# mic-rud/Learned-Compression-of-Point-Cloud-Geometry-and-Attributes

Measured on AMD Instinct MI355X. Metric: encode+decode Mpoints/sec, higher is better.
Workload: dtype f32

## Files before the change

include/pcc_hip.h:

```cpp
#ifndef PCC_HIP_H
#define PCC_HIP_H

#include <stdint.h>

#ifdef __cplusplus
extern "C" {
#endif

#define PCC_OK 0
#define PCC_ERR_ARG (-1)
#define PCC_ERR_HIP (-2)
#define PCC_ERR_UNSUPPORTED (-3)
#define PCC_ERR_DATA (-4)

#define PCC_ACT_NONE 0
#define PCC_ACT_RELU 1
#define PCC_ACT_LEAKY_RELU 2

int pcc_version(void);
const char* pcc_last_error(void);
int pcc_device_count(void);
int pcc_device_name(int dev, char* out, int out_len);

int64_t pcc_hash_capacity(int64_t n);
// ... 34 lines not shown
int64_t pcc_small_map_max(void);
int32_t pcc_small_paths(int32_t mask);
int pcc_small_kernel_map(const int32_t* out_coords, int64_t n_out, const uint64_t* in_keys, const int32_t* in_vals, int64_t in_cap,
                         int32_t ksize, int32_t step, int32_t sign, int32_t* nbr, uint32_t* row_mask, int32_t* order,
                         uint32_t* group_mask32, void* scratch, int64_t scratch_bytes, void* stream);

int64_t pcc_conv_packed_elems(int32_t K, int32_t cin, int32_t cout);
int pcc_conv_pack_weights(const float* w, int32_t K, int32_t cin, int32_t cout, float* w_packed,
                          void* stream);
int pcc_conv_fwd(const float* fin, int64_t n_in, int32_t cin, const float* w, const float* w_packed,
                 const float* bias, const int32_t* nbr, const int32_t* order,
                 const uint32_t* group_mask32, int32_t K, float* fout, int64_t n_out, int32_t cout,
                 int32_t act, const float* film, const float* residual, void* stream);

int64_t pcc_conv_small_max(int64_t workgroups);

int pcc_conv_kernel_name(int32_t mode, int64_t n_in, int32_t cin, int32_t cout, int64_t n_out, int32_t K, int32_t has_nbr,
                         char* buf, int32_t len);

int64_t pcc_conv_packed_elems_bf16(int32_t K, int32_t cin, int32_t cout);
int pcc_conv_pack_weights_bf16(const float* w, int32_t K, int32_t cin, int32_t cout, uint16_t* w_packed, void* stream);
int pcc_conv_fwd_bf16(const uint16_t* fin, int64_t n_in, int32_t cin, const uint16_t* w_packed, const float* bias,
                      const int32_t* nbr, const int32_t* order, const uint32_t* group_mask32, int32_t K, float* fout,
                      int64_t n_out, int32_t cout, int32_t act, const float* film, const float* residual, void* stream);

int pcc_epilogue_fwd(const float* c, const float* film, const float* residual, int64_t n, int32_t channels, int32_t act,
                     float* out, void* stream);
int pcc_epilogue_bwd(const float* dout, const float* c, const float* film, int64_t n, int32_t channels, int32_t act,
                     float* dc, float* dfilm, void* stream);

// ... 118 lines not shown
```

learned-compression-of-point-cloud-geometry-and-attributes_amd/_lib.py:

```python
import ctypes
import os
import subprocess

_HERE = os.path.dirname(os.path.abspath(__file__))
SO_PATH = os.path.join(_HERE, "libpcc_hip.so")
_lib = None

c_void_p, c_int, c_i32, c_i64 = ctypes.c_void_p, ctypes.c_int, ctypes.c_int32, ctypes.c_int64

SIGNATURES = {
    "pcc_version": (c_int, []),
    "pcc_last_error": (ctypes.c_char_p, []),
    "pcc_device_count": (c_int, []),
    "pcc_device_name": (c_int, [c_int, ctypes.c_char_p, c_int]),
    "pcc_hash_capacity": (c_i64, [c_i64]),
    "pcc_hash_build": (c_int, [c_void_p, c_i64, c_void_p, c_void_p, c_i64, c_i32, c_void_p, c_void_p]),
    "pcc_hash_lookup": (c_int, [c_void_p, c_void_p, c_i64, c_i32, c_void_p, c_i64, c_void_p, c_void_p]),
    "pcc_scan_scratch_elems": (c_i64, [c_i64]),
    "pcc_stride_map": (c_int, [c_void_p, c_i64, c_i32, c_void_p, c_void_p, c_i64, c_void_p, c_void_p, c_void_p, c_void_p]),
    "pcc_children": (c_int, [c_void_p, c_i64, c_i32, c_i32, c_void_p, c_void_p, c_i64, c_void_p, c_void_p, c_void_p, c_void_p]),
    "pcc_kernel_map": (c_int, [c_void_p, c_i64, c_void_p, c_void_p, c_i64, c_i32, c_i32, c_i32, c_void_p, c_void_p, c_void_p, c_void_p]),
    "pcc_pair_count": (c_int, [c_void_p, c_i64, c_void_p, c_void_p]),
    "pcc_conv_packed_elems": (c_i64, [c_i32, c_i32, c_i32]),
    "pcc_conv_pack_weights": (c_int, [c_void_p, c_i32, c_i32, c_i32, c_void_p, c_void_p]),
    "pcc_order_scratch_bytes": (c_i64, [c_i64]),
    "pcc_order_rows_by_mask": (c_int, [c_void_p, c_void_p, c_i64, c_i32, c_i32, c_void_p, c_void_p, c_void_p, c_i64, c_void_p]),
    "pcc_permute_map_rows": (c_int, [c_void_p, c_void_p, c_i64, c_i32, c_void_p, c_void_p]),
    "pcc_conv_fwd": (c_int, [c_void_p, c_i64, c_i32, c_void_p, c_void_p, c_void_p, c_void_p, c_void_p, c_void_p, c_i32,
                             c_void_p, c_i64, c_i32, c_i32, c_void_p, c_void_p, c_void_p]),
    "pcc_conv_small_max": (c_i64, [c_i64]),
    "pcc_conv_kernel_name": (c_int, [c_i32, c_i64, c_i32, c_i32, c_i64, c_i32, c_i32, ctypes.c_char_p, c_i32]),
    "pcc_small_map_max": (c_i64, []),
    "pcc_small_paths": (c_i32, [c_i32]),
    "pcc_small_kernel_map": (c_int, [c_void_p, c_i64, c_void_p, c_void_p, c_i64, c_i32, c_i32, c_i32, c_void_p, c_void_p, c_void_p,
                                     c_void_p, c_void_p, c_i64, c_void_p]),
    "pcc_conv_packed_elems_bf16": (c_i64, [c_i32, c_i32, c_i32]),
    "pcc_conv_pack_weights_bf16": (c_int, [c_void_p, c_i32, c_i32, c_i32, c_void_p, c_void_p]),
    "pcc_conv_fwd_bf16": (c_int, [c_void_p, c_i64, c_i32, c_void_p, c_void_p, c_void_p, c_void_p, c_void_p, c_i32, c_void_p, c_i64,
                                  c_i32, c_i32, c_void_p, c_void_p, c_void_p]),
    "pcc_conv_packed_elems_x3": (c_i64, [c_i32, c_i32, c_i32]),
    "pcc_conv_pack_weights_x3": (c_int, [c_void_p, c_i32, c_i32, c_i32, c_void_p, c_void_p]),
    "pcc_conv_fwd_x3": (c_int, [c_void_p, c_i64, c_i32, c_void_p, c_void_p, c_void_p, c_void_p, c_void_p, c_i32, c_void_p, c_i64,
                                c_i32, c_i32, c_void_p, c_void_p, c_void_p]),
    "pcc_epilogue_fwd": (c_int, [c_void_p, c_void_p, c_void_p, c_i64, c_i32, c_i32, c_void_p, c_void_p]),
    "pcc_cast_colsum_scratch_elems": (c_i64, [c_i32]),
# ... 211 lines not shown
```

learned-compression-of-point-cloud-geometry-and-attributes_amd/csrc/conv.hip:

```cpp
#include <stdlib.h>

#include <type_traits>

#include "common.h"

namespace pcc {

typedef float f32x2 __attribute__((ext_vector_type(2)));
typedef float f32x4 __attribute__((ext_vector_type(4)));
typedef float f32x16 __attribute__((ext_vector_type(16)));
typedef __bf16 bf16x8 __attribute__((ext_vector_type(8)));

struct ConvArgs {
    const float* fin;
    const float* w;
    const float* wp;
    const float* bias;
    const int32_t* nbr;
    const int32_t* order;
    const uint32_t* gmask;
    float* fout;
    const float* film;
    const float* residual;
    int64_t n_in, n_out;
// ... 68 lines not shown
        wp[((base + 0 * 4 + g) * coutp + col) * 8 + j] = hi;
        wp[((base + 1 * 4 + g) * coutp + col) * 8 + j] = mid;
        wp[((base + 2 * 4 + g) * coutp + col) * 8 + j] = lo;
    }
}

constexpr int A_LD_DMA = 32;

template <int BM, int BN, bool X3 = false>
constexpr int conv_lds_bytes() { return 2 * (BM * A_LD_DMA + (X3 ? 12 : 8) * BN * 4) * (int)sizeof(float); }

__device__ float g_zero_line[256] = {0.0f};

typedef __attribute__((address_space(3))) void* lds_ptr_t;
typedef const __attribute__((address_space(1))) void* gbl_ptr_t;

template <int BM, int BN, int WAVES_M, int WAVES_N, bool HAS_NBR>
__global__ __launch_bounds__(256) void conv_mfma_kernel(const ConvArgs a) {
    constexpr int RPT = BM / 32;
    constexpr int WM = BM / WAVES_M, WN = BN / WAVES_N;
    constexpr int MT = WM / 32, NT = WN / 32;
    constexpr int A_LD = A_LD_DMA;
    constexpr int A_ELEMS = BM * A_LD;
    constexpr int W_ELEMS = 8 * BN * 4;
    constexpr int W_LOADS = (8 * BN) / 256;
    static_assert(WAVES_M * WAVES_N == 4 && MT >= 1 && NT >= 1 && W_LOADS >= 1, "bad tiling");

    extern __shared__ __attribute__((aligned(16))) float smem[];
    float* As = smem;
    float* Ws = smem + 2 * A_ELEMS;
// ... 232 lines not shown
    constexpr int W_ELEMS = (X3 ? 12 : 8) * BN * 4;
    constexpr int W_LOADS = ((X3 ? 12 : 8) * BN) / 256;
    static_assert(WAVES_M * WAVES_N == 4 && MT >= 1 && MT <= 2 && NT >= 1 && W_LOADS >= 1, "bad tiling");
    static_assert(!(BF16 && X3), "one operand mode at a time");
    constexpr int ESZ = BF16 ? 2 : 4;

    extern __shared__ __attribute__((aligned(16))) float smem[];
    float* As = smem;
    float* Ws = smem + 2 * A_ELEMS;

    const int t = threadIdx.x;
    const int lane = t & 63, wid = t >> 6;
    const int r = lane & 31, h = lane >> 5;
    const int wrow = (wid / WAVES_N) * WM, wcol = (wid % WAVES_N) * WN;

    const int ntiles_n = a.coutp / BN;
    const int64_t tile = blockIdx.x / ntiles_n;
    const int nt = blockIdx.x - (int)(tile * ntiles_n);
    const int64_t row0 = tile * BM;
    const int K = a.K;

    uint32_t tmask, mmask[MT];
    {
        const uint32_t all = (K >= 32) ? 0xffffffffu : ((1u << K) - 1u);
        if (a.gmask) {
            const int64_t g0 = row0 >> 5;
            const int64_t ng = (a.n_out + 31) >> 5;
            tmask = 0u;
#pragma unroll
            for (int g = 0; g < BM / 32; ++g) tmask |= (g0 + g < ng) ? (a.gmask[g0 + g] & all) : 0u;
#pragma unroll
            for (int m = 0; m < MT; ++m) {
                const int64_t g = g0 + (wrow >> 5) + m;
                const uint32_t v = (g < ng) ? (a.gmask[g] & all) : 0u;
                mmask[m] = __builtin_amdgcn_readfirstlane(v);
            }
        } else {
            tmask = all;
#pragma unroll
            for (int m = 0; m < MT; ++m) mmask[m] = all;
        }
        tmask = __builtin_amdgcn_readfirstlane(tmask);
    }

    f32x16 acc[MT][NT];
#pragma unroll
    for (int m = 0; m < MT; ++m)
#pragma unroll
        for (int n = 0; n < NT; ++n) {
#pragma unroll
            for (int i = 0; i < 16; ++i) acc[m][n][i] = 0.0f;
        }

    if (tmask != 0u) {
        __amdgpu_buffer_rsrc_t rsrc_a = __builtin_amdgcn_make_buffer_rsrc(
            const_cast<float*>(a.fin), 0, (int)(uint32_t)(a.n_in * a.cin * ESZ), BUF_FLAGS);
        __amdgpu_buffer_rsrc_t rsrc_w = __builtin_amdgcn_make_buffer_rsrc(
            const_cast<float*>(a.wp), 0, (int)((uint32_t)K * a.cin * a.coutp * (X3 ? 6 : ESZ)), BUF_FLAGS);
        __amdgpu_buffer_rsrc_t rsrc_n = __builtin_amdgcn_make_buffer_rsrc(
            const_cast<int32_t*>(a.nbr), 0, HAS_NBR ? (int)(uint32_t)(a.n_out * K * 4) : 0, BUF_FLAGS);

        const int gchunk = t & 7;
        uint32_t q16[RPT], n_voff[RPT], a_voff[RPT];
        int idx_nxt[RPT];
        bool rvalid[RPT];
#pragma unroll
        for (int i = 0; i < RPT; ++i) {
            const int grow = wid * (BM / 4) + 8 * i + (lane >> 3);
            const int64_t pos = row0 + grow;
            rvalid[i] = pos < a.n_out;
            const int64_t ps = rvalid[i] ? pos : a.n_out - 1;
            q16[i] = (uint32_t)((gchunk ^ ((grow >> 1) & 7)) * 16);
            n_voff[i] = (uint32_t)(((HAS_NBR && a.order) ? (int64_t)a.order[ps] : ps) * K * 4);
            idx_nxt[i] = (int)ps;
        }
        uint32_t w_voff[W_LOADS];
#pragma unroll
        for (int j = 0; j < W_LOADS; ++j) {
            const int f = t + 256 * j;
            const int g = f / BN, col = f - g * BN;
            w_voff[j] = (uint32_t)((g * a.coutp + nt * BN + col) * 16);
        }
        const int wave_u = __builtin_amdgcn_readfirstlane(wid);
        const uint32_t w_kstride = X3 ? (uint32_t)(a.cin / 32) * 12u * a.coutp * 16u
                                      : (uint32_t)(a.cin * ESZ / 16) * a.coutp * 16;
        const uint32_t w_cstride = (uint32_t)(X3 ? 12 : 8) * a.coutp * 16;
        const uint32_t a_row_bytes = (uint32_t)a.cin * ESZ;

        auto load_idx = [&](int k) {
            if constexpr (HAS_NBR) {
#pragma unroll
                for (int i = 0; i < RPT; ++i)
                    idx_nxt[i] = (int)__builtin_amdgcn_raw_buffer_load_b32(rsrc_n, n_voff[i], k * 4, 0);
            }
        };
        auto set_src = [&](bool real) {
#pragma unroll
            for (int i = 0; i < RPT; ++i) {
                const bool ok = real && rvalid[i] && idx_nxt[i] >= 0;
                a_voff[i] = ok ? (uint32_t)idx_nxt[i] * a_row_bytes + q16[i] : BUF_OOB;
            }
        };
        auto dma = [&](int k, auto cc, auto bufc) {
            constexpr int c = decltype(cc)::value;
            constexpr int buf = decltype(bufc)::value;
#pragma unroll
            for (int i = 0; i < RPT; ++i)
                __builtin_amdgcn_raw_ptr_buffer_load_lds(rsrc_a, (lds_ptr_t)(As + buf * A_ELEMS + (wave_u * RPT + i) * 256), 16,
                                                         a_voff[i], c * 128, 0, 0);
            const uint32_t wso = (uint32_t)k * w_kstride + (uint32_t)c * w_cstride;
#pragma unroll
            for (int j = 0; j < W_LOADS; ++j)
                __builtin_amdgcn_raw_ptr_buffer_load_lds(rsrc_w, (lds_ptr_t)(Ws + buf * W_ELEMS + (wave_u * 64 + 256 * j) * 4), 16,
                                                         w_voff[j], wso, 0, 0);
        };

        const int sw = (r >> 1) & 7;
        uint32_t a_addr[2][4], w_addr[2];
#pragma unroll
        for (int b = 0; b < 2; ++b) {
#pragma unroll
            for (int kk = 0; kk < 4; ++kk)
                a_addr[b][kk] = (uint32_t)((b * A_ELEMS + (wrow + r) * 32 + (((kk ^ (sw >> 1)) << 1) | (h ^ (sw & 1))) * 4) * 4);
            w_addr[b] = (uint32_t)((2 * A_ELEMS + b * W_ELEMS + (h * BN + wcol + r) * 4) * 4);
        }
        auto lds4 = [&](uint32_t addr) { return *reinterpret_cast<const f32x4*>(reinterpret_cast<const char*>(smem) + addr); };

        uint32_t a3_addr[2][2][2];
#pragma unroll
        for (int b = 0; b < 2; ++b)
#pragma unroll
            for (int q = 0; q < 2; ++q)
#pragma unroll
                for (int e = 0; e < 2; ++e)
                    a3_addr[b][q][e] = (uint32_t)((b * A_ELEMS + (wrow + r) * 32 + ((4 * q + 2 * h + e) ^ sw) * 4) * 4);
        auto split8 = [&](const f32x4& lo4, const f32x4& hi4, bf16x8& ph, bf16x8& pm, bf16x8& pl) {
            uint32_t hb[8], mb[8], lb[8];
#pragma unroll
            for (int j = 0; j < 8; ++j) {
                const float x = j < 4 ? lo4[j] : hi4[j - 4];
                hb[j] = __float_as_uint(x) & 0xFFFF0000u;
                const float r1 = x - __uint_as_float(hb[j]);
                mb[j] = __float_as_uint(r1) & 0xFFFF0000u;
                lb[j] = __float_as_uint(r1 - __uint_as_float(mb[j]));
            }
            typedef uint32_t u32x4 __attribute__((ext_vector_type(4)));
            u32x4 vh, vm, vl;
#pragma unroll
            for (int d = 0; d < 4; ++d) {
                vh[d] = __builtin_amdgcn_perm(hb[2 * d + 1], hb[2 * d], 0x07060302u);
                vm[d] = __builtin_amdgcn_perm(mb[2 * d + 1], mb[2 * d], 0x07060302u);
                vl[d] = __builtin_amdgcn_perm(lb[2 * d + 1], lb[2 * d], 0x07060302u);
            }
            ph = __builtin_bit_cast(bf16x8, vh);
            pm = __builtin_bit_cast(bf16x8, vm);
            pl = __builtin_bit_cast(bf16x8, vl);
        };
        auto compute_live_x3 = [&](auto bufc, auto live_tag) {
            constexpr int buf = decltype(bufc)::value;
            constexpr unsigned LIVE = decltype(live_tag)::value;
            __builtin_amdgcn_s_setprio(1);
#pragma unroll
            for (int q = 0; q < 2; ++q) {
                bf16x8 ah[MT], am[MT], al[MT];
#pragma unroll
                for (int m = 0; m < MT; ++m)
                    if ((LIVE >> m) & 1u)
                        split8(lds4(a3_addr[buf][q][0] + 32 * m * 32 * 4), lds4(a3_addr[buf][q][1] + 32 * m * 32 * 4), ah[m], am[m], al[m]);
                bf16x8 bh[NT], bm[NT], bl[NT];
#pragma unroll
                for (int n = 0; n < NT; ++n) {
                    const uint32_t wb = w_addr[buf] + (uint32_t)((2 * q * BN + 32 * n) * 16);
                    bh[n] = __builtin_bit_cast(bf16x8, lds4(wb));
                    bm[n] = __builtin_bit_cast(bf16x8, lds4(wb + 4 * BN * 16));
                    bl[n] = __builtin_bit_cast(bf16x8, lds4(wb + 8 * BN * 16));
                }
#define PCC_X3_TERM(A, B)                                                                                                   \
    _Pragma("unroll") for (int m = 0; m < MT; ++m) _Pragma("unroll") for (int n = 0; n < NT; ++n) if ((LIVE >> m) & 1u)     \
        acc[m][n] = __builtin_amdgcn_mfma_f32_32x32x16_bf16(A[m], B[n], acc[m][n], 0, 0, 0)
                PCC_X3_TERM(al, bh);
                PCC_X3_TERM(ah, bl);
                PCC_X3_TERM(am, bm);
                PCC_X3_TERM(am, bh);
                PCC_X3_TERM(ah, bm);
                PCC_X3_TERM(ah, bh);
#undef PCC_X3_TERM
            }
            __builtin_amdgcn_s_setprio(0);
        };
        auto compute_live = [&](auto bufc, auto live_tag) {
            if constexpr (X3) {
                compute_live_x3(bufc, live_tag);
                return;
            }
            constexpr int buf = decltype(bufc)::value;
            constexpr unsigned LIVE = decltype(live_tag)::value;
            f32x4 av[2][MT], bv[2][NT];
            __builtin_amdgcn_s_setprio(1);
#pragma unroll
            for (int m = 0; m < MT; ++m)
                if ((LIVE >> m) & 1u) av[0][m] = lds4(a_addr[buf][0] + 32 * m * 32 * 4);
#pragma unroll
            for (int n = 0; n < NT; ++n) bv[0][n] = lds4(w_addr[buf] + 32 * n * 16);
#pragma unroll
            for (int kk = 0; kk < 4; ++kk) {
                const int cb = kk & 1, nb = cb ^ 1;
                if (kk + 1 < 4) {
#pragma unroll
                    for (int m = 0; m < MT; ++m)
                        if ((LIVE >> m) & 1u) av[nb][m] = lds4(a_addr[buf][kk + 1] + 32 * m * 32 * 4);
#pragma unroll
                    for (int n = 0; n < NT; ++n) bv[nb][n] = lds4(w_addr[buf] + (2 * (kk + 1) * BN + 32 * n) * 16);
                }
                if constexpr (BF16) {
#pragma unroll
                    for (int m = 0; m < MT; ++m)
#pragma unroll
                        for (int n = 0; n < NT; ++n)
                            if ((LIVE >> m) & 1u)
                                acc[m][n] = __builtin_amdgcn_mfma_f32_32x32x16_bf16(__builtin_bit_cast(bf16x8, av[cb][m]),
                                                                                    __builtin_bit_cast(bf16x8, bv[cb][n]), acc[m][n], 0, 0, 0);
                } else {
#pragma unroll
                    for (int s = 0; s < 4; ++s)
#pragma unroll
                        for (int m = 0; m < MT; ++m)
#pragma unroll
                            for (int n = 0; n < NT; ++n)
                                if ((LIVE >> m) & 1u)
                                    acc[m][n] = __builtin_amdgcn_mfma_f32_32x32x2f32(av[cb][m][s], bv[cb][n][s], acc[m][n], 0, 0, 0);
                }
            }
            __builtin_amdgcn_s_setprio(0);
        };
        auto compute = [&](auto bufc, unsigned live) {
            if constexpr (MT == 1) {
                if (live) compute_live(bufc, std::integral_constant<unsigned, 1u>{});
            } else {
                if (live == 3u) compute_live(bufc, std::integral_constant<unsigned, 3u>{});
                else if (live == 1u) compute_live(bufc, std::integral_constant<unsigned, 1u>{});
                else if (live == 2u) compute_live(bufc, std::integral_constant<unsigned, 2u>{});
            }
        };

        uint32_t rem = tmask;
        int k = __builtin_ctz(rem);
        rem &= rem - 1u;
        auto offset_body = [&](auto pc) {
            constexpr int P = decltype(pc)::value;
            const int knext = rem ? __builtin_ctz(rem) : -1;
            const uint32_t rem2 = rem & (rem - 1u);
            const int kn2 = rem2 ? __builtin_ctz(rem2) : (knext >= 0 ? knext : k);
            unsigned live = 0;
#pragma unroll
            for (int m = 0; m < MT; ++m) live |= ((mmask[m] >> k) & 1u) << m;
            static_for<0, CCH>([&](auto cc) {
                constexpr int c = decltype(cc)::value;
                constexpr int buf = (P + c) & 1;
                if constexpr (c + 1 < CCH) {
                    dma(k, std::integral_constant<int, c + 1>{}, std::integral_constant<int, buf ^ 1>{});
                } else {
                    set_src(knext >= 0);
                    dma(knext >= 0 ? knext : k, std::integral_constant<int, 0>{}, std::integral_constant<int, buf ^ 1>{});
                    load_idx(kn2);
                }
                compute(std::integral_constant<int, buf>{}, live);
                __syncthreads();
            });
            const bool more = knext >= 0;
            k = more ? knext : k;
            rem = rem2;
            return more;
        };

        load_idx(k);
        set_src(true);
        dma(k, std::integral_constant<int, 0>{}, std::integral_constant<int, 0>{});
        load_idx(rem ? __builtin_ctz(rem) : k);
        __syncthreads();
        while (true) {
            if (!offset_body(std::integral_constant<int, 0>{})) break;
            if constexpr (CCH & 1) {
                if (!offset_body(std::integral_constant<int, 1>{})) break;
            }
        }
    }

#pragma unroll
    for (int m = 0; m < MT; ++m) {
#pragma unroll
        for (int n = 0; n < NT; ++n) {
#pragma unroll
            for (int reg = 0; reg < 16; ++reg) {
                const int col = nt * BN + wcol + 32 * n + r;
                if (col >= a.cout) continue;
                const float bcol = a.bias ? a.bias[col] : 0.0f;
                const int64_t pos = row0 + wrow + 32 * m + (reg & 3) + 8 * (reg >> 2) + 4 * h;
                if (pos >= a.n_out) continue;
                const int64_t row = a.order ? a.order[pos] : pos;
                float v = acc[m][n][reg] + bcol;
                if (a.film) {
                    const float* fr = a.film + row * (2 * (int64_t)a.cout);
                    v = v * fr[col] + fr[a.cout + col];
                }
                v = apply_act(v, a.act);
                if (a.residual) v += a.residual[row * a.cout + col];
                a.fout[row * a.cout + col] = v;
            }
        }
    }
#endif
}

template <int SC, int NS>
constexpr int conv_small_lds_bytes() { return (NS * SC * (32 * 32 + 8 * 32 * 4) + 32 * 32) * (int)sizeof(float); }

template <int SC, int NS>
__global__ __launch_bounds__(512) void conv_small_kernel(const ConvArgs a) {
#if defined(__HIP_DEVICE_COMPILE__)
    constexpr int A_STAGE = SC * 32 * 32;
    constexpr int W_STAGE = SC * 8 * 32 * 4;
    constexpr int STAGE = A_STAGE + W_STAGE;
    constexpr int DMAS = 2 * SC;
    static_assert(NS >= 2 && (NS - 1) * DMAS <= 63, "vmcnt is a 6-bit counter");
// ... 390 lines not shown
        PCC_REQUIRE((uint64_t)a.n_in * a.cin * 4 <= BUF_OOB && (uint64_t)a.n_out * a.K * 4 <= BUF_OOB &&
                    (uint64_t)a.K * a.cin * a.coutp * 6 <= BUF_OOB, "%s: operands of 4 GiB and more are not supported", who);
    }
    const int64_t wgs128 = ((a.n_out + 63) / 64) * (a.coutp / 128);
    auto tile = [&](int bm, int bn, int wm, int wn) { p.bm = bm; p.bn = bn; p.wm = wm; p.wn = wn; return PCC_OK; };
    if (wide && wgs128 < FILL_WGS) return tile(64, 64, 2, 2);
    if (wide && mode == CONV_F32 && wgs128 < ROW32_MAX_WGS) return tile(32, 128, 1, 4);
    if (wide) return tile(64, 128, 2, 2);
    if (a.coutp % 64 == 0) return mode == CONV_X3 ? tile(64, 64, 2, 2) : tile(128, 64, 2, 2);
    if (mode != CONV_X3) return tile(128, 32, 4, 1);
    pcc::set_error("%s: cout=%d not supported (output width rounded up to 32 must be a multiple of 64)", who, a.cout);
    return PCC_ERR_UNSUPPORTED;
}

template <auto KERN>
static int launch(int64_t blocks, int threads, size_t lds, size_t lds_limit, const ConvArgs& a, hipStream_t st) {
    static bool limit_set = false;
    if (lds_limit && !limit_set) {
        PCC_CHECK_HIP(hipFuncSetAttribute(reinterpret_cast<const void*>(KERN), hipFuncAttributeMaxDynamicSharedMemorySize, (int)lds_limit));
        limit_set = true;
    }
    PCC_REQUIRE(blocks < (1ll << 31), "conv: grid too large");
    hipLaunchKernelGGL(KERN, dim3((unsigned)blocks), dim3(threads), lds, st, a);
    PCC_LAUNCH_CHECK();
    return PCC_OK;
}

template <ConvMode M, int BM, int BN, int WM, int WN, int CCH>
static int launch_buf(int64_t blocks, const ConvArgs& a, hipStream_t st) {
    constexpr bool BF16 = M == CONV_BF16, X3 = M == CONV_X3;
    if constexpr (BF16 && CCH > 4) {
        return PCC_ERR_UNSUPPORTED;
    } else {
        constexpr int lds = conv_lds_bytes<BM, BN, X3>();
        return a.nbr ? launch<conv_mfma_buf_kernel<BM, BN, WM, WN, CCH, true, BF16, X3>>(blocks, 256, lds, lds, a, st)
                     : launch<conv_mfma_buf_kernel<BM, BN, WM, WN, CCH, false, BF16, X3>>(blocks, 256, lds, lds, a, st);
    }
}

template <ConvMode M, int BM, int BN, int WM, int WN>
static int launch_mfma(const ConvPlan& p, const ConvArgs& a, hipStream_t st) {
    const int64_t blocks = (a.n_out + BM - 1) / BM * (a.coutp / BN);
    if constexpr (M == CONV_F32) {
        if (p.family == FAM_GLOBAL) {
            constexpr int lds = conv_lds_bytes<BM, BN>();
            return a.nbr ? launch<conv_mfma_kernel<BM, BN, WM, WN, true>>(blocks, 256, lds, lds, a, st)
                         : launch<conv_mfma_kernel<BM, BN, WM, WN, false>>(blocks, 256, lds, lds, a, st);
        }
    }
    switch (p.cch) {
        case 1: return launch_buf<M, BM, BN, WM, WN, 1>(blocks, a, st);
// ... 171 lines not shown
    else if (K == 27 && al16 && cout == 4) PCC_GS27(4);
    else
#undef PCC_GS27
        hipLaunchKernelGGL(gather_sum_kernel, dim3(blocks_for(n_out * cout, 256, 1 << 20)), dim3(256), 0, as_stream(stream),
                           scores, ld, nbr, K, cout, bias, out, n_out, act);
    PCC_LAUNCH_CHECK();
    return PCC_OK;
}

int64_t pcc_conv_small_max(int64_t workgroups) {
    const int64_t before = small_max_value();
    if (workgroups >= 0) g_small_max = workgroups;
    return before;
}

int pcc_conv_fwd(const float* fin, int64_t n_in, int32_t cin, const float* w, const float* w_packed, const float* bias,
                 const int32_t* nbr, const int32_t* order, const uint32_t* group_mask32, int32_t K, float* fout,
                 int64_t n_out, int32_t cout, int32_t act, const float* film, const float* residual, void* stream) {
    return conv_fwd(CONV_F32, {fin, w, w_packed, bias, nbr, order, group_mask32, fout, film, residual, n_in, n_out, cin, cout,
                               round_up32(cout), K, act, 0}, stream);
}

int pcc_conv_kernel_name(int32_t mode, int64_t n_in, int32_t cin, int32_t cout, int64_t n_out, int32_t K, int32_t has_nbr,
                         char* buf, int32_t len) {
    PCC_REQUIRE(mode >= CONV_F32 && mode <= CONV_X3, "pcc_conv_kernel_name: bad mode %d", mode);
    static const int32_t any_map = 0;
    ConvArgs a = {};
    a.nbr = has_nbr ? &any_map : nullptr;
    a.n_in = n_in; a.n_out = n_out; a.cin = cin; a.cout = cout; a.coutp = round_up32(cout); a.K = K;
    const ConvMode m = ConvMode(mode);
// ... 15 lines not shown
```

Measured before the change: 8.974.

## Make buffered MFMA conv kernel a grid-stride loop with cross-tile prefetch

Restructures the buffered MFMA sparse-conv kernel so each workgroup loops over several output tiles. It stages the next tile's group masks, order indices and first neighbour index while the current tile computes, and keeps LDS double-buffer images flipping across tiles. A launcher can cap the grid at a CU-filling count from an occupancy query or a user-set limit, but conv_streams_tiles returns false, so by default the grid still equals the tile count unless a maximum is set. The aim is to hide per-tile prologue latency and launch overhead, at the cost of more registers and more complex control flow.

```diff
diff --git a/include/pcc_hip.h b/include/pcc_hip.h
--- a/include/pcc_hip.h
+++ b/include/pcc_hip.h
@@ -72,6 +72,8 @@
                  int32_t act, const float* film, const float* residual, void* stream);
 
 int64_t pcc_conv_small_max(int64_t workgroups);
+
+int64_t pcc_conv_max_workgroups(int64_t workgroups);
 
 int pcc_conv_kernel_name(int32_t mode, int64_t n_in, int32_t cin, int32_t cout, int64_t n_out, int32_t K, int32_t has_nbr,
                          char* buf, int32_t len);
diff --git a/learned-compression-of-point-cloud-geometry-and-attributes_amd/_lib.py b/learned-compression-of-point-cloud-geometry-and-attributes_amd/_lib.py
--- a/learned-compression-of-point-cloud-geometry-and-attributes_amd/_lib.py
+++ b/learned-compression-of-point-cloud-geometry-and-attributes_amd/_lib.py
@@ -29,6 +29,7 @@
     "pcc_conv_fwd": (c_int, [c_void_p, c_i64, c_i32, c_void_p, c_void_p, c_void_p, c_void_p, c_void_p, c_void_p, c_i32,
                              c_void_p, c_i64, c_i32, c_i32, c_void_p, c_void_p, c_void_p]),
     "pcc_conv_small_max": (c_i64, [c_i64]),
+    "pcc_conv_max_workgroups": (c_i64, [c_i64]),
     "pcc_conv_kernel_name": (c_int, [c_i32, c_i64, c_i32, c_i32, c_i64, c_i32, c_i32, ctypes.c_char_p, c_i32]),
     "pcc_small_map_max": (c_i64, []),
     "pcc_small_paths": (c_i32, [c_i32]),
diff --git a/learned-compression-of-point-cloud-geometry-and-attributes_amd/csrc/conv.hip b/learned-compression-of-point-cloud-geometry-and-attributes_amd/csrc/conv.hip
--- a/learned-compression-of-point-cloud-geometry-and-attributes_amd/csrc/conv.hip
+++ b/learned-compression-of-point-cloud-geometry-and-attributes_amd/csrc/conv.hip
@@ -106,6 +106,7 @@
 
 typedef __attribute__((address_space(3))) void* lds_ptr_t;
 typedef const __attribute__((address_space(1))) void* gbl_ptr_t;
+typedef const __attribute__((address_space(4))) struct ConvArgs* karg_ptr_t;
 
 template <int BM, int BN, int WAVES_M, int WAVES_N, bool HAS_NBR>
 __global__ __launch_bounds__(256) void conv_mfma_kernel(const ConvArgs a) {
@@ -368,300 +369,395 @@
     const int r = lane & 31, h = lane >> 5;
     const int wrow = (wid / WAVES_N) * WM, wcol = (wid % WAVES_N) * WN;
 
-    const int ntiles_n = a.coutp / BN;
-    const int64_t tile = blockIdx.x / ntiles_n;
-    const int nt = blockIdx.x - (int)(tile * ntiles_n);
-    const int64_t row0 = tile * BM;
     const int K = a.K;
-
-    uint32_t tmask, mmask[MT];
-    {
-        const uint32_t all = (K >= 32) ? 0xffffffffu : ((1u << K) - 1u);
-        if (a.gmask) {
-            const int64_t g0 = row0 >> 5;
-            const int64_t ng = (a.n_out + 31) >> 5;
-            tmask = 0u;
-#pragma unroll
-            for (int g = 0; g < BM / 32; ++g) tmask |= (g0 + g < ng) ? (a.gmask[g0 + g] & all) : 0u;
-#pragma unroll
-            for (int m = 0; m < MT; ++m) {
-                const int64_t g = g0 + (wrow >> 5) + m;
-                const uint32_t v = (g < ng) ? (a.gmask[g] & all) : 0u;
-                mmask[m] = __builtin_amdgcn_readfirstlane(v);
-            }
-        } else {
-            tmask = all;
-#pragma unroll
-            for (int m = 0; m < MT; ++m) mmask[m] = all;
-        }
-        tmask = __builtin_amdgcn_readfirstlane(tmask);
-    }
+    const uint32_t all = (K >= 32) ? 0xffffffffu : ((1u << K) - 1u);
+    const uint32_t ntiles_n = (uint32_t)(a.coutp / BN);
+    const uint32_t n_out = (uint32_t)a.n_out;
+    const uint32_t items = ((n_out + BM - 1) / BM) * ntiles_n;
+    const uint32_t G = gridDim.x;
+    const uint32_t ng = (n_out + 31) >> 5;
+
+    __amdgpu_buffer_rsrc_t rsrc_a = __builtin_amdgcn_make_buffer_rsrc(
+        const_cast<float*>(a.fin), 0, (int)(uint32_t)(a.n_in * a.cin * ESZ), BUF_FLAGS);
+    __amdgpu_buffer_rsrc_t rsrc_w = __builtin_amdgcn_make_buffer_rsrc(
+        const_cast<float*>(a.wp), 0, (int)((uint32_t)K * a.cin * a.coutp * (X3 ? 6 : ESZ)), BUF_FLAGS);
+    __amdgpu_buffer_rsrc_t rsrc_n = __builtin_amdgcn_make_buffer_rsrc(
+        const_cast<int32_t*>(a.nbr), 0, HAS_NBR ? (int)(uint32_t)(a.n_out * K * 4) : 0, BUF_FLAGS);
+
+    const int gchunk = t & 7;
+    int grow[RPT];
+    uint32_t q16[RPT];
+#pragma unroll
+    for (int i = 0; i < RPT; ++i) {
+        grow[i] = wid * (BM / 4) + 8 * i + (lane >> 3);
+        q16[i] = (uint32_t)((gchunk ^ ((grow[i] >> 1) & 7)) * 16);
+    }
+    uint32_t w_voff[W_LOADS];
+#pragma unroll
+    for (int j = 0; j < W_LOADS; ++j) {
+        const int f = t + 256 * j;
+        const int g = f / BN, col = f - g * BN;
+        w_voff[j] = (uint32_t)((g * a.coutp + col) * 16);
+    }
+    const int wave_u = __builtin_amdgcn_readfirstlane(wid);
+    const uint32_t w_kstride = X3 ? (uint32_t)(a.cin / 32) * 12u * a.coutp * 16u
+                                  : (uint32_t)(a.cin * ESZ / 16) * a.coutp * 16;
+    const uint32_t w_cstride = (uint32_t)(X3 ? 12 : 8) * a.coutp * 16;
+    const uint32_t a_row_bytes = (uint32_t)a.cin * ESZ;
+
+    struct Raw {
+        uint32_t gm[BM / 32];
+        int32_t ord[RPT];
+    };
+    struct Tile {
+        uint32_t row0;
+        uint32_t ncol;
+        uint32_t tmask, mmask[MT];
+        uint32_t n_voff[RPT];
+        int idx[RPT];
+    };
+    auto first_k = [](uint32_t m) { return m ? __builtin_ctz(m) : 0; };
+    auto second_k = [](uint32_t m) { return (m & (m - 1u)) ? __builtin_ctz(m & (m - 1u)) : (m ? __builtin_ctz(m) : 0); };
+    const bool has_gm = a.gmask != nullptr, has_ord = a.order != nullptr;
+    const uint32_t* const gm_src = has_gm ? a.gmask : reinterpret_cast<const uint32_t*>(a.wp);
+    const int32_t* const ord_src = has_ord ? a.order : reinterpret_cast<const int32_t*>(a.wp);
+    auto stage_a = [&](uint32_t item, Raw& rw) {
+        const uint32_t it = item < items ? item : items - 1;
+        const uint32_t tile = __builtin_amdgcn_readfirstlane(it / ntiles_n);
+#pragma unroll
+        for (int g = 0; g < BM / 32; ++g) {
+            const uint32_t gi = tile * (BM / 32) + g;
+            rw.gm[g] = gm_src[has_gm ? (gi < ng ? gi : ng - 1) : 0];
+        }
+        if constexpr (HAS_NBR) {
+#pragma unroll
+            for (int i = 0; i < RPT; ++i) {
+                const uint32_t pos = tile * BM + grow[i];
+                rw.ord[i] = ord_src[has_ord ? (pos < n_out ? pos : n_out - 1) : 0];
+            }
+        }
+    };
+    auto stage_b = [&](uint32_t item, const Raw& rw, Tile& tl) {
+        const bool valid = item < items;
+        const uint32_t it = valid ? item : items - 1;
+        const uint32_t tile = __builtin_amdgcn_readfirstlane(it / ntiles_n);
+        tl.row0 = tile * BM;
+        tl.ncol = (it - tile * ntiles_n) * BN;
+        uint32_t tm = 0u, mm[MT];
+#pragma unroll
+        for (int m = 0; m < MT; ++m) mm[m] = 0u;
+#pragma unroll
+        for (int g = 0; g < BM / 32; ++g) {
+            const uint32_t v = has_gm ? ((tile * (BM / 32) + g < ng) ? (rw.gm[g] & all) : 0u) : all;
+            tm |= v;
+#pragma unroll
+            for (int m = 0; m < MT; ++m) mm[m] = (g == (wrow >> 5) + m) ? v : mm[m];
+        }
+        tl.tmask = valid ? __builtin_amdgcn_readfirstlane(tm) : 0u;
+#pragma unroll
+        for (int m = 0; m < MT; ++m) tl.mmask[m] = mm[m];
+        const int k0 = first_k(tl.tmask);
+#pragma unroll
+        for (int i = 0; i < RPT; ++i) {
+            const uint32_t pos = tl.row0 + grow[i];
+            const uint32_t ps = pos < n_out ? pos : n_out - 1;
+            tl.n_voff[i] = ((HAS_NBR && has_ord) ? (uint32_t)rw.ord[i] : ps) * (uint32_t)(K * 4);
+            if constexpr (HAS_NBR) tl.idx[i] = (int)__builtin_amdgcn_raw_buffer_load_b32(rsrc_n, tl.n_voff[i], k0 * 4, 0);
+            else tl.idx[i] = (int)ps;
+        }
+    };
+
+    uint32_t a_voff[RPT];
+    int idx_nxt[RPT];
+    int flip = 0;
+    auto dma = [&](int k, uint32_t ncol, auto cc, auto bufc) {
+        constexpr int c = decltype(cc)::value;
+        constexpr int buf = decltype(bufc)::value;
+        int img = flip;
+        asm volatile("" : "+s"(img));
+        img ^= buf;
+#pragma unroll
+        for (int i = 0; i < RPT; ++i)
+            __builtin_amdgcn_raw_ptr_buffer_load_lds(rsrc_a, (lds_ptr_t)(As + img * A_ELEMS + (wave_u * RPT + i) * 256), 16,
+                                                     a_voff[i], c * 128, 0, 0);
+        const uint32_t wso = __builtin_amdgcn_readfirstlane((uint32_t)k * w_kstride + (uint32_t)c * w_cstride + ncol * 16u);
+#pragma unroll
+        for (int j = 0; j < W_LOADS; ++j)
+            __builtin_amdgcn_raw_ptr_buffer_load_lds(rsrc_w, (lds_ptr_t)(Ws + img * W_ELEMS + (wave_u * 64 + 256 * j) * 4), 16,
+                                                     w_voff[j], wso, 0, 0);
+    };
+
+    const int sw = (r >> 1) & 7;
+    uint32_t a_addr[2][4], w_addr[2];
+#pragma unroll
+    for (int b = 0; b < 2; ++b) {
+#pragma unroll
+        for (int kk = 0; kk < 4; ++kk)
+            a_addr[b][kk] = (uint32_t)((b * A_ELEMS + (wrow + r) * 32 + (((kk ^ (sw >> 1)) << 1) | (h ^ (sw & 1))) * 4) * 4);
+        w_addr[b] = (uint32_t)((2 * A_ELEMS + b * W_ELEMS + (h * BN + wcol + r) * 4) * 4);
+    }
+    auto lds4 = [&](uint32_t addr) { return *reinterpret_cast<const f32x4*>(reinterpret_cast<const char*>(smem) + addr); };
+
+    uint32_t a3_addr[2][2][2];
+#pragma unroll
+    for (int b = 0; b < 2; ++b)
+#pragma unroll
+        for (int q = 0; q < 2; ++q)
+#pragma unroll
+            for (int e = 0; e < 2; ++e)
+                a3_addr[b][q][e] = (uint32_t)((b * A_ELEMS + (wrow + r) * 32 + ((4 * q + 2 * h + e) ^ sw) * 4) * 4);
+    auto swap_images = [&]() {
+        flip ^= 1;
+#pragma unroll
+        for (int kk = 0; kk < 4; ++kk) { const uint32_t x = a_addr[0][kk]; a_addr[0][kk] = a_addr[1][kk]; a_addr[1][kk] = x; }
+        { const uint32_t x = w_addr[0]; w_addr[0] = w_addr[1]; w_addr[1] = x; }
+        if constexpr (X3) {
+#pragma unroll
+            for (int q = 0; q < 2; ++q)
+#pragma unroll
+                for (int e = 0; e < 2; ++e) { const uint32_t x = a3_addr[0][q][e]; a3_addr[0][q][e] = a3_addr[1][q][e]; a3_addr[1][q][e] = x; }
+        }
+    };
+    auto split8 = [&](const f32x4& lo4, const f32x4& hi4, bf16x8& ph, bf16x8& pm, bf16x8& pl) {
+        uint32_t hb[8], mb[8], lb[8];
+#pragma unroll
+        for (int j = 0; j < 8; ++j) {
+            const float x = j < 4 ? lo4[j] : hi4[j - 4];
+            hb[j] = __float_as_uint(x) & 0xFFFF0000u;
+            const float r1 = x - __uint_as_float(hb[j]);
+            mb[j] = __float_as_uint(r1) & 0xFFFF0000u;
+            lb[j] = __float_as_uint(r1 - __uint_as_float(mb[j]));
+        }
+        typedef uint32_t u32x4 __attribute__((ext_vector_type(4)));
+        u32x4 vh, vm, vl;
+#pragma unroll
+        for (int d = 0; d < 4; ++d) {
+            vh[d] = __builtin_amdgcn_perm(hb[2 * d + 1], hb[2 * d], 0x07060302u);
+            vm[d] = __builtin_amdgcn_perm(mb[2 * d + 1], mb[2 * d], 0x07060302u);
+            vl[d] = __builtin_amdgcn_perm(lb[2 * d + 1], lb[2 * d], 0x07060302u);
+        }
+        ph = __builtin_bit_cast(bf16x8, vh);
+        pm = __builtin_bit_cast(bf16x8, vm);
+        pl = __builtin_bit_cast(bf16x8, vl);
+    };
 
     f32x16 acc[MT][NT];
-#pragma unroll
-    for (int m = 0; m < MT; ++m)
-#pragma unroll
-        for (int n = 0; n < NT; ++n) {
-#pragma unroll
-            for (int i = 0; i < 16; ++i) acc[m][n][i] = 0.0f;
-        }
-
-    if (tmask != 0u) {
-        __amdgpu_buffer_rsrc_t rsrc_a = __builtin_amdgcn_make_buffer_rsrc(
-            const_cast<float*>(a.fin), 0, (int)(uint32_t)(a.n_in * a.cin * ESZ), BUF_FLAGS);
-        __amdgpu_buffer_rsrc_t rsrc_w = __builtin_amdgcn_make_buffer_rsrc(
-            const_cast<float*>(a.wp), 0, (int)((uint32_t)K * a.cin * a.coutp * (X3 ? 6 : ESZ)), BUF_FLAGS);
-        __amdgpu_buffer_rsrc_t rsrc_n = __builtin_amdgcn_make_buffer_rsrc(
-            const_cast<int32_t*>(a.nbr), 0, HAS_NBR ? (int)(uint32_t)(a.n_out * K * 4) : 0, BUF_FLAGS);
-
-        const int gchunk = t & 7;
-        uint32_t q16[RPT], n_voff[RPT], a_voff[RPT];
-        int idx_nxt[RPT];
-        bool rvalid[RPT];
-#pragma unroll
-        for (int i = 0; i < RPT; ++i) {
-            const int grow = wid * (BM / 4) + 8 * i + (lane >> 3);
-            const int64_t pos = row0 + grow;
-            rvalid[i] = pos < a.n_out;
-            const int64_t ps = rvalid[i] ? pos : a.n_out - 1;
-            q16[i] = (uint32_t)((gchunk ^ ((grow >> 1) & 7)) * 16);
-            n_voff[i] = (uint32_t)(((HAS_NBR && a.order) ? (int64_t)a.order[ps] : ps) * K * 4);
-            idx_nxt[i] = (int)ps;
-        }
-        uint32_t w_voff[W_LOADS];
-#pragma unroll
-        for (int j = 0; j < W_LOADS; ++j) {
-            const int f = t + 256 * j;
-            const int g = f / BN, col = f - g * BN;
-            w_voff[j] = (uint32_t)((g * a.coutp + nt * BN + col) * 16);
-        }
-        const int wave_u = __builtin_amdgcn_readfirstlane(wid);
-        const uint32_t w_kstride = X3 ? (uint32_t)(a.cin / 32) * 12u * a.coutp * 16u
-                                      : (uint32_t)(a.cin * ESZ / 16) * a.coutp * 16;
-        const uint32_t w_cstride = (uint32_t)(X3 ? 12 : 8) * a.coutp * 16;
-        const uint32_t a_row_bytes = (uint32_t)a.cin * ESZ;
-
-        auto load_idx = [&](int k) {
-            if constexpr (HAS_NBR) {
-#pragma unroll
-                for (int i = 0; i < RPT; ++i)
-                    idx_nxt[i] = (int)__builtin_amdgcn_raw_buffer_load_b32(rsrc_n, n_voff[i], k * 4, 0);
-            }
-        };
-        auto set_src = [&](bool real) {
-#pragma unroll
-            for (int i = 0; i < RPT; ++i) {
-                const bool ok = real && rvalid[i] && idx_nxt[i] >= 0;
-                a_voff[i] = ok ? (uint32_t)idx_nxt[i] * a_row_bytes + q16[i] : BUF_OOB;
-            }
-        };
-        auto dma = [&](int k, auto cc, auto bufc) {
-            constexpr int c = decltype(cc)::value;
-            constexpr int buf = decltype(bufc)::value;
-#pragma unroll
-            for (int i = 0; i < RPT; ++i)
-                __builtin_amdgcn_raw_ptr_buffer_load_lds(rsrc_a, (lds_ptr_t)(As + buf * A_ELEMS + (wave_u * RPT + i) * 256), 16,
-                                                         a_voff[i], c * 128, 0, 0);
-            const uint32_t wso = (uint32_t)k * w_kstride + (uint32_t)c * w_cstride;
-#pragma unroll
-            for (int j = 0; j < W_LOADS; ++j)
-                __builtin_amdgcn_raw_ptr_buffer_load_lds(rsrc_w, (lds_ptr_t)(Ws + buf * W_ELEMS + (wave_u * 64 + 256 * j) * 4), 16,
-                                                         w_voff[j], wso, 0, 0);
-        };
-
-        const int sw = (r >> 1) & 7;
-        uint32_t a_addr[2][4], w_addr[2];
-#pragma unroll
-        for (int b = 0; b < 2; ++b) {
-#pragma unroll
-            for (int kk = 0; kk < 4; ++kk)
-                a_addr[b][kk] = (uint32_t)((b * A_ELEMS + (wrow + r) * 32 + (((kk ^ (sw >> 1)) << 1) | (h ^ (sw & 1))) * 4) * 4);
-            w_addr[b] = (uint32_t)((2 * A_ELEMS + b * W_ELEMS + (h * BN + wcol + r) * 4) * 4);
-        }
-        auto lds4 = [&](uint32_t addr) { return *reinterpret_cast<const f32x4*>(reinterpret_cast<const char*>(smem) + addr); };
-
-        uint32_t a3_addr[2][2][2];
-#pragma unroll
-        for (int b = 0; b < 2; ++b)
-#pragma unroll
-            for (int q = 0; q < 2; ++q)
-#pragma unroll
-                for (int e = 0; e < 2; ++e)
-                    a3_addr[b][q][e] = (uint32_t)((b * A_ELEMS + (wrow + r) * 32 + ((4 * q + 2 * h + e) ^ sw) * 4) * 4);
-        auto split8 = [&](const f32x4& lo4, const f32x4& hi4, bf16x8& ph, bf16x8& pm, bf16x8& pl) {
-            uint32_t hb[8], mb[8], lb[8];
-#pragma unroll
-            for (int j = 0; j < 8; ++j) {
-                const float x = j < 4 ? lo4[j] : hi4[j - 4];
-                hb[j] = __float_as_uint(x) & 0xFFFF0000u;
-                const float r1 = x - __uint_as_float(hb[j]);
-                mb[j] = __float_as_uint(r1) & 0xFFFF0000u;
-                lb[j] = __float_as_uint(r1 - __uint_as_float(mb[j]));
-            }
-            typedef uint32_t u32x4 __attribute__((ext_vector_type(4)));
-            u32x4 vh, vm, vl;
-#pragma unroll
-            for (int d = 0; d < 4; ++d) {
-                vh[d] = __builtin_amdgcn_perm(hb[2 * d + 1], hb[2 * d], 0x07060302u);
-                vm[d] = __builtin_amdgcn_perm(mb[2 * d + 1], mb[2 * d], 0x07060302u);
-                vl[d] = __builtin_amdgcn_perm(lb[2 * d + 1], lb[2 * d], 0x07060302u);
-            }
-            ph = __builtin_bit_cast(bf16x8, vh);
-            pm = __builtin_bit_cast(bf16x8, vm);
-            pl = __builtin_bit_cast(bf16x8, vl);
-        };
-        auto compute_live_x3 = [&](auto bufc, auto live_tag) {
-            constexpr int buf = decltype(bufc)::value;
-            constexpr unsigned LIVE = decltype(live_tag)::value;
-            __builtin_amdgcn_s_setprio(1);
-#pragma unroll
-            for (int q = 0; q < 2; ++q) {
-                bf16x8 ah[MT], am[MT], al[MT];
-#pragma unroll
-                for (int m = 0; m < MT; ++m)
-                    if ((LIVE >> m) & 1u)
-                        split8(lds4(a3_addr[buf][q][0] + 32 * m * 32 * 4), lds4(a3_addr[buf][q][1] + 32 * m * 32 * 4), ah[m], am[m], al[m]);
-                bf16x8 bh[NT], bm[NT], bl[NT];
-#pragma unroll
-                for (int n = 0; n < NT; ++n) {
-                    const uint32_t wb = w_addr[buf] + (uint32_t)((2 * q * BN + 32 * n) * 16);
-                    bh[n] = __builtin_bit_cast(bf16x8, lds4(wb));
-                    bm[n] = __builtin_bit_cast(bf16x8, lds4(wb + 4 * BN * 16));
-                    bl[n] = __builtin_bit_cast(bf16x8, lds4(wb + 8 * BN * 16));
-                }
+    auto compute_live_x3 = [&](auto bufc, auto live_tag) {
+        constexpr int buf = decltype(bufc)::value;
+        constexpr unsigned LIVE = decltype(live_tag)::value;
+        __builtin_amdgcn_s_setprio(1);
+#pragma unroll
+        for (int q = 0; q < 2; ++q) {
+            bf16x8 ah[MT], am[MT], al[MT];
+#pragma unroll
+            for (int m = 0; m < MT; ++m)
+                if ((LIVE >> m) & 1u)
+                    split8(lds4(a3_addr[buf][q][0] + 32 * m * 32 * 4), lds4(a3_addr[buf][q][1] + 32 * m * 32 * 4), ah[m], am[m], al[m]);
+            bf16x8 bh[NT], bm[NT], bl[NT];
+#pragma unroll
+            for (int n = 0; n < NT; ++n) {
+                const uint32_t wb = w_addr[buf] + (uint32_t)((2 * q * BN + 32 * n) * 16);
+                bh[n] = __builtin_bit_cast(bf16x8, lds4(wb));
+                bm[n] = __builtin_bit_cast(bf16x8, lds4(wb + 4 * BN * 16));
+                bl[n] = __builtin_bit_cast(bf16x8, lds4(wb + 8 * BN * 16));
+            }
 #define PCC_X3_TERM(A, B)                                                                                                   \
     _Pragma("unroll") for (int m = 0; m < MT; ++m) _Pragma("unroll") for (int n = 0; n < NT; ++n) if ((LIVE >> m) & 1u)     \
         acc[m][n] = __builtin_amdgcn_mfma_f32_32x32x16_bf16(A[m], B[n], acc[m][n], 0, 0, 0)
-                PCC_X3_TERM(al, bh);
-                PCC_X3_TERM(ah, bl);
-                PCC_X3_TERM(am, bm);
-                PCC_X3_TERM(am, bh);
-                PCC_X3_TERM(ah, bm);
-                PCC_X3_TERM(ah, bh);
+            PCC_X3_TERM(al, bh);
+            PCC_X3_TERM(ah, bl);
+            PCC_X3_TERM(am, bm);
+            PCC_X3_TERM(am, bh);
+            PCC_X3_TERM(ah, bm);
+            PCC_X3_TERM(ah, bh);
 #undef PCC_X3_TERM
-            }
-            __builtin_amdgcn_s_setprio(0);
-        };
-        auto compute_live = [&](auto bufc, auto live_tag) {
-            if constexpr (X3) {
-                compute_live_x3(bufc, live_tag);
-                return;
-            }
-            constexpr int buf = decltype(bufc)::value;
-            constexpr unsigned LIVE = decltype(live_tag)::value;
-            f32x4 av[2][MT], bv[2][NT];
-            __builtin_amdgcn_s_setprio(1);
-#pragma unroll
-            for (int m = 0; m < MT; ++m)
-                if ((LIVE >> m) & 1u) av[0][m] = lds4(a_addr[buf][0] + 32 * m * 32 * 4);
-#pragma unroll
-            for (int n = 0; n < NT; ++n) bv[0][n] = lds4(w_addr[buf] + 32 * n * 16);
-#pragma unroll
-            for (int kk = 0; kk < 4; ++kk) {
-                const int cb = kk & 1, nb = cb ^ 1;
-                if (kk + 1 < 4) {
-#pragma unroll
-                    for (int m = 0; m < MT; ++m)
-                        if ((LIVE >> m) & 1u) av[nb][m] = lds4(a_addr[buf][kk + 1] + 32 * m * 32 * 4);
-#pragma unroll
-                    for (int n = 0; n < NT; ++n) bv[nb][n] = lds4(w_addr[buf] + (2 * (kk + 1) * BN + 32 * n) * 16);
-                }
-                if constexpr (BF16) {
+        }
+        __builtin_amdgcn_s_setprio(0);
+    };
+    auto compute_live = [&](auto bufc, auto live_tag) {
+        if constexpr (X3) {
+            compute_live_x3(bufc, live_tag);
+            return;
+        }
+        constexpr int buf = decltype(bufc)::value;
+        constexpr unsigned LIVE = decltype(live_tag)::value;
+        f32x4 av[2][MT], bv[2][NT];
+        __builtin_amdgcn_s_setprio(1);
+#pragma unroll
+        for (int m = 0; m < MT; ++m)
+            if ((LIVE >> m) & 1u) av[0][m] = lds4(a_addr[buf][0] + 32 * m * 32 * 4);
+#pragma unroll
+        for (int n = 0; n < NT; ++n) bv[0][n] = lds4(w_addr[buf] + 32 * n * 16);
+#pragma unroll
+        for (int kk = 0; kk < 4; ++kk) {
+            const int cb = kk & 1, nb = cb ^ 1;
+            if (kk + 1 < 4) {
+#pragma unroll
+                for (int m = 0; m < MT; ++m)
+                    if ((LIVE >> m) & 1u) av[nb][m] = lds4(a_addr[buf][kk + 1] + 32 * m * 32 * 4);
+#pragma unroll
+                for (int n = 0; n < NT; ++n) bv[nb][n] = lds4(w_addr[buf] + (2 * (kk + 1) * BN + 32 * n) * 16);
+            }
+            if constexpr (BF16) {
+#pragma unroll
+                for (int m = 0; m < MT; ++m)
+#pragma unroll
+                    for (int n = 0; n < NT; ++n)
+                        if ((LIVE >> m) & 1u)
+                            acc[m][n] = __builtin_amdgcn_mfma_f32_32x32x16_bf16(__builtin_bit_cast(bf16x8, av[cb][m]),
+                                                                                __builtin_bit_cast(bf16x8, bv[cb][n]), acc[m][n], 0, 0, 0);
+            } else {
+#pragma unroll
+                for (int s = 0; s < 4; ++s)
 #pragma unroll
                     for (int m = 0; m < MT; ++m)
 #pragma unroll
                         for (int n = 0; n < NT; ++n)
                             if ((LIVE >> m) & 1u)
-                                acc[m][n] = __builtin_amdgcn_mfma_f32_32x32x16_bf16(__builtin_bit_cast(bf16x8, av[cb][m]),
-                                                                                    __builtin_bit_cast(bf16x8, bv[cb][n]), acc[m][n], 0, 0, 0);
-                } else {
-#pragma unroll
-                    for (int s = 0; s < 4; ++s)
-#pragma unroll
-                        for (int m = 0; m < MT; ++m)
-#pragma unroll
-                            for (int n = 0; n < NT; ++n)
-                                if ((LIVE >> m) & 1u)
-                                    acc[m][n] = __builtin_amdgcn_mfma_f32_32x32x2f32(av[cb][m][s], bv[cb][n][s], acc[m][n], 0, 0, 0);
+                                acc[m][n] = __builtin_amdgcn_mfma_f32_32x32x2f32(av[cb][m][s], bv[cb][n][s], acc[m][n], 0, 0, 0);
+            }
+        }
+        __builtin_amdgcn_s_setprio(0);
+    };
+    auto compute = [&](auto bufc, unsigned live) {
+        if constexpr (MT == 1) {
+            if (live) compute_live(bufc, std::integral_constant<unsigned, 1u>{});
+        } else {
+            if (live == 3u) compute_live(bufc, std::integral_constant<unsigned, 3u>{});
+            else if (live == 1u) compute_live(bufc, std::integral_constant<unsigned, 1u>{});
+            else if (live == 2u) compute_live(bufc, std::integral_constant<unsigned, 2u>{});
+        }
+    };
+
+    uint32_t item = blockIdx.x;
+    Tile cur, nxt;
+    Raw raw;
+    {
+        Raw first;
+        stage_a(item, first);
+        stage_a(item + G, raw);
+        stage_b(item, first, cur);
+    }
+    bool primed = false;
+    while (true) {
+        stage_b(item + G, raw, nxt);
+        stage_a(item + 2 * G, raw);
+
+#pragma unroll
+        for (int m = 0; m < MT; ++m)
+#pragma unroll
+            for (int n = 0; n < NT; ++n) {
+#pragma unroll
+                for (int i = 0; i < 16; ++i) acc[m][n][i] = 0.0f;
+            }
+
+        if (cur.tmask != 0u) {
+            int k = first_k(cur.tmask);
+            uint32_t mmask[MT];
+#pragma unroll
+            for (int m = 0; m < MT; ++m) mmask[m] = __builtin_amdgcn_readfirstlane(cur.mmask[m]);
+            uint32_t rem = cur.tmask & (cur.tmask - 1u);
+            if (!primed) {
+#pragma unroll
+                for (int i = 0; i < RPT; ++i)
+                    a_voff[i] = (cur.row0 + grow[i] < n_out && cur.idx[i] >= 0) ? (uint32_t)cur.idx[i] * a_row_bytes + q16[i] : BUF_OOB;
+                dma(k, cur.ncol, std::integral_constant<int, 0>{}, std::integral_constant<int, 0>{});
+#pragma unroll
+                for (int i = 0; i < RPT; ++i) {
+                    if constexpr (HAS_NBR) idx_nxt[i] = (int)__builtin_amdgcn_raw_buffer_load_b32(rsrc_n, cur.n_voff[i], second_k(cur.tmask) * 4, 0);
                 }
-            }
-            __builtin_amdgcn_s_setprio(0);
-        };
-        auto compute = [&](auto bufc, unsigned live) {
-            if constexpr (MT == 1) {
-                if (live) compute_live(bufc, std::integral_constant<unsigned, 1u>{});
+                __syncthreads();
+            }
+            if constexpr (!HAS_NBR) {
+#pragma unroll
+                for (int i = 0; i < RPT; ++i) idx_nxt[i] = cur.idx[i];
+            }
+            const bool pf = nxt.tmask != 0u;
+
+            auto offset_body = [&]() {
+                const int knext = rem ? __builtin_ctz(rem) : -1;
+                const uint32_t rem2 = rem & (rem - 1u);
+                const bool more = knext >= 0;
+                const int kd = more ? knext : (pf ? first_k(nxt.tmask) : k);
+                const int ki = more ? (rem2 ? __builtin_ctz(rem2) : knext) : second_k(nxt.tmask);
+                const uint32_t ncol_d = more ? cur.ncol : nxt.ncol;
+                const uint32_t row0_d = (more || !pf) ? cur.row0 : nxt.row0;
+                unsigned live = 0;
+#pragma unroll
+                for (int m = 0; m < MT; ++m) live |= ((mmask[m] >> k) & 1u) << m;
+                static_for<0, CCH>([&](auto cc) {
+                    constexpr int c = decltype(cc)::value;
+                    constexpr int buf = c & 1;
+                    if constexpr (c + 1 < CCH) {
+                        dma(k, cur.ncol, std::integral_constant<int, c + 1>{}, std::integral_constant<int, buf ^ 1>{});
+                    } else {
+#pragma unroll
+                        for (int i = 0; i < RPT; ++i) {
+                            const int idx = more ? idx_nxt[i] : nxt.idx[i];
+                            const bool ok = (more || pf) && row0_d + grow[i] < n_out && idx >= 0;
+                            a_voff[i] = ok ? (uint32_t)idx * a_row_bytes + q16[i] : BUF_OOB;
+                        }
+                        dma(kd, ncol_d, std::integral_constant<int, 0>{}, std::integral_constant<int, buf ^ 1>{});
+                        if constexpr (HAS_NBR) {
+#pragma unroll
+                            for (int i = 0; i < RPT; ++i)
+                                idx_nxt[i] = (int)__builtin_amdgcn_raw_buffer_load_b32(rsrc_n, more ? cur.n_voff[i] : nxt.n_voff[i], ki * 4, 0);
+                        }
+                    }
+                    compute(std::integral_constant<int, buf>{}, live);
+                    __syncthreads();
+                });
+                k = more ? knext : k;
+                rem = rem2;
+                return more;
+            };
+
+            if constexpr (CCH & 1) {
+                while (offset_body()) swap_images();
+                swap_images();
             } else {
-                if (live == 3u) compute_live(bufc, std::integral_constant<unsigned, 3u>{});
-                else if (live == 1u) compute_live(bufc, std::integral_constant<unsigned, 1u>{});
-                else if (live == 2u) compute_live(bufc, std::integral_constant<unsigned, 2u>{});
-            }
-        };
-
-        uint32_t rem = tmask;
-        int k = __builtin_ctz(rem);
-        rem &= rem - 1u;
-        auto offset_body = [&](auto pc) {
-            constexpr int P = decltype(pc)::value;
-            const int knext = rem ? __builtin_ctz(rem) : -1;
-            const uint32_t rem2 = rem & (rem - 1u);
-            const int kn2 = rem2 ? __builtin_ctz(rem2) : (knext >= 0 ? knext : k);
-            unsigned live = 0;
-#pragma unroll
-            for (int m = 0; m < MT; ++m) live |= ((mmask[m] >> k) & 1u) << m;
-            static_for<0, CCH>([&](auto cc) {
-                constexpr int c = decltype(cc)::value;
-                constexpr int buf = (P + c) & 1;
-                if constexpr (c + 1 < CCH) {
-                    dma(k, std::integral_constant<int, c + 1>{}, std::integral_constant<int, buf ^ 1>{});
-                } else {
-                    set_src(knext >= 0);
-                    dma(knext >= 0 ? knext : k, std::integral_constant<int, 0>{}, std::integral_constant<int, buf ^ 1>{});
-                    load_idx(kn2);
+                while (offset_body()) {}
+            }
+            primed = pf;
+        }
+
+        int erow = wrow + 4 * h, ecol = wcol + r;
+        asm volatile("" : "+v"(erow), "+v"(ecol));
+        karg_ptr_t ea = (karg_ptr_t)__builtin_amdgcn_kernarg_segment_ptr();
+        asm volatile("" : "+s"(ea));
+        const float* const e_bias = ea->bias;
+        const float* const e_film = ea->film;
+        const float* const e_res = ea->residual;
+        const int32_t* const e_order = ea->order;
+        float* const e_fout = ea->fout;
+        const int e_cout = ea->cout, e_act = ea->act;
+#pragma unroll
+        for (int m = 0; m < MT; ++m) {
+#pragma unroll
+            for (int n = 0; n < NT; ++n) {
+#pragma unroll
+                for (int reg = 0; reg < 16; ++reg) {
+                    const int col = (int)cur.ncol + ecol + 32 * n;
+                    if (col >= e_cout) continue;
+                    const float bcol = e_bias ? e_bias[col] : 0.0f;
+                    const uint32_t pos = cur.row0 + erow + 32 * m + (reg & 3) + 8 * (reg >> 2);
+                    if (pos >= n_out) continue;
+                    const int64_t row = e_order ? e_order[pos] : pos;
+                    float v = acc[m][n][reg] + bcol;
+                    if (e_film) {
+                        const float* fr = e_film + row * (2 * (int64_t)e_cout);
+                        v = v * fr[col] + fr[e_cout + col];
+                    }
+                    v = apply_act(v, e_act);
+                    if (e_res) v += e_res[row * e_cout + col];
+                    e_fout[row * e_cout + col] = v;
                 }
-                compute(std::integral_constant<int, buf>{}, live);
-                __syncthreads();
-            });
-            const bool more = knext >= 0;
-            k = more ? knext : k;
-            rem = rem2;
-            return more;
-        };
-
-        load_idx(k);
-        set_src(true);
-        dma(k, std::integral_constant<int, 0>{}, std::integral_constant<int, 0>{});
-        load_idx(rem ? __builtin_ctz(rem) : k);
-        __syncthreads();
-        while (true) {
-            if (!offset_body(std::integral_constant<int, 0>{})) break;
-            if constexpr (CCH & 1) {
-                if (!offset_body(std::integral_constant<int, 1>{})) break;
-            }
-        }
-    }
-
-#pragma unroll
-    for (int m = 0; m < MT; ++m) {
-#pragma unroll
-        for (int n = 0; n < NT; ++n) {
-#pragma unroll
-            for (int reg = 0; reg < 16; ++reg) {
-                const int col = nt * BN + wcol + 32 * n + r;
-                if (col >= a.cout) continue;
-                const float bcol = a.bias ? a.bias[col] : 0.0f;
-                const int64_t pos = row0 + wrow + 32 * m + (reg & 3) + 8 * (reg >> 2) + 4 * h;
-                if (pos >= a.n_out) continue;
-                const int64_t row = a.order ? a.order[pos] : pos;
-                float v = acc[m][n][reg] + bcol;
-                if (a.film) {
-                    const float* fr = a.film + row * (2 * (int64_t)a.cout);
-                    v = v * fr[col] + fr[a.cout + col];
-                }
-                v = apply_act(v, a.act);
-                if (a.residual) v += a.residual[row * a.cout + col];
-                a.fout[row * a.cout + col] = v;
-            }
-        }
+            }
+        }
+
+        item += G;
+        if (item >= items) break;
+        cur = nxt;
     }
 #endif
 }
@@ -1082,16 +1178,56 @@
 }
 
 template <auto KERN>
-static int launch(int64_t blocks, int threads, size_t lds, size_t lds_limit, const ConvArgs& a, hipStream_t st) {
+static int raise_lds_limit(size_t lds_limit) {
     static bool limit_set = false;
     if (lds_limit && !limit_set) {
         PCC_CHECK_HIP(hipFuncSetAttribute(reinterpret_cast<const void*>(KERN), hipFuncAttributeMaxDynamicSharedMemorySize, (int)lds_limit));
         limit_set = true;
     }
+    return PCC_OK;
+}
+
+template <auto KERN>
+static int launch(int64_t blocks, int threads, size_t lds, size_t lds_limit, const ConvArgs& a, hipStream_t st) {
+    const int rc = raise_lds_limit<KERN>(lds_limit);
+    if (rc != PCC_OK) return rc;
     PCC_REQUIRE(blocks < (1ll << 31), "conv: grid too large");
     hipLaunchKernelGGL(KERN, dim3((unsigned)blocks), dim3(threads), lds, st, a);
     PCC_LAUNCH_CHECK();
     return PCC_OK;
+}
+
+template <ConvMode M, int BM, int BN>
+constexpr bool conv_streams_tiles() { return false; }
+
+static int64_t g_max_wgs = 0;
+
+template <auto KERN>
+static int stream_grid(size_t lds, int64_t& grid) {
+    static int64_t fill = 0;
+    if (!fill) {
+        int dev = 0, cus = 0, per_cu = 0;
+        PCC_CHECK_HIP(hipGetDevice(&dev));
+        PCC_CHECK_HIP(hipDeviceGetAttribute(&cus, hipDeviceAttributeMultiprocessorCount, dev));
+        PCC_CHECK_HIP(hipOccupancyMaxActiveBlocksPerMultiprocessor(&per_cu, reinterpret_cast<const void*>(KERN), 256, lds));
+        PCC_REQUIRE(cus > 0 && per_cu > 0, "conv: the occupancy query gives %d workgroups on %d CUs", per_cu, cus);
+        fill = (int64_t)cus * per_cu;
+    }
+    grid = fill;
+    return PCC_OK;
+}
+
+template <auto KERN, bool STREAMS>
+static int launch_tiles(int64_t tiles, size_t lds, const ConvArgs& a, hipStream_t st) {
+    PCC_REQUIRE(tiles < (1ll << 30), "conv: too many tiles");
+    int rc = raise_lds_limit<KERN>(lds);
+    if (rc != PCC_OK) return rc;
+    int64_t grid = tiles;
+    if (g_max_wgs > 0) grid = g_max_wgs;
+    else if (STREAMS && (rc = stream_grid<KERN>(lds, grid)) != PCC_OK) return rc;
+    if (grid >= tiles) grid = tiles;
+    else if (grid > 8) grid -= grid % 8;
+    return launch<KERN>(grid, 256, lds, lds, a, st);
 }
 
 template <ConvMode M, int BM, int BN, int WM, int WN, int CCH>
@@ -1101,8 +1237,9 @@
         return PCC_ERR_UNSUPPORTED;
     } else {
         constexpr int lds = conv_lds_bytes<BM, BN, X3>();
-        return a.nbr ? launch<conv_mfma_buf_kernel<BM, BN, WM, WN, CCH, true, BF16, X3>>(blocks, 256, lds, lds, a, st)
-                     : launch<conv_mfma_buf_kernel<BM, BN, WM, WN, CCH, false, BF16, X3>>(blocks, 256, lds, lds, a, st);
+        constexpr bool S = conv_streams_tiles<M, BM, BN>();
+        return a.nbr ? launch_tiles<conv_mfma_buf_kernel<BM, BN, WM, WN, CCH, true, BF16, X3>, S>(blocks, lds, a, st)
+                     : launch_tiles<conv_mfma_buf_kernel<BM, BN, WM, WN, CCH, false, BF16, X3>, S>(blocks, lds, a, st);
     }
 }
 
@@ -1304,6 +1441,12 @@
     return before;
 }
 
+int64_t pcc_conv_max_workgroups(int64_t workgroups) {
+    const int64_t before = g_max_wgs;
+    if (workgroups >= 0) g_max_wgs = workgroups;
+    return before;
+}
+
 int pcc_conv_fwd(const float* fin, int64_t n_in, int32_t cin, const float* w, const float* w_packed, const float* bias,
                  const int32_t* nbr, const int32_t* order, const uint32_t* group_mask32, int32_t K, float* fout,
                  int64_t n_out, int32_t cout, int32_t act, const float* film, const float* residual, void* stream) {
```

Result: slower. 8.833 (-1.6%).
